# willSapgreen/stereo-vision

Hardware: AMD Instinct MI355X
Metric: stereo pairs/sec (ELAS 1242x375, ROBOTICS, D1+D2+LR) (higher is better)
Workload: dtype u8

## Files before the change

### stereo-vision_amd/csrc/elas_kernels.hip

```cpp
#include <hip/hip_runtime.h>

#include <algorithm>
#include <cstdlib>

#include "dev_common.h"
#include "prior_core.h"
#include "svh_internal.h"

namespace svh {

namespace {

constexpr int kWave = 64;

template <int kCtrl, int kRowMask>
__device__ __forceinline__ uint32_t dpp_min_step(uint32_t v) {
    const uint32_t o =
        (uint32_t)__builtin_amdgcn_update_dpp((int)0xFFFFFFFFu, (int)v, kCtrl, kRowMask, 0xF, false);
    return o < v ? o : v;
}

__device__ __forceinline__ uint32_t wave_min_u32(uint32_t v) {
    v = dpp_min_step<0xB1, 0xF>(v);
    v = dpp_min_step<0x4E, 0xF>(v);
// ... 1679 lines not shown
    __syncthreads();
    float* D = out.D[side] + (size_t)pair * out.stride[side] + (size_t)y * P.DW;
    const int16_t* other = s_raw + (1 - side) * Q.Wr;
    if (P.sub) {
        for (int x = x0; x < P.DW; x += half) {
            const int d = raw_row[x];
            float o = -10.f;
            const float fd = (float)d, step = fd / 2, uwf = side ? (float)x + step : (float)x - step;
            if (d >= 0 && uwf >= 0 && uwf < (float)P.DW)
                if (!(fabsf((float)other[(int)uwf] - fd) > lr_threshold)) o = fd;
            D[x] = o;
        }
        return;
    }
    const int ithr = lr_threshold >= 0.f ? (int)fminf(floorf(lr_threshold), 1048576.f) : -1;
    const uint32_t span = ithr >= 0 ? 2u * (uint32_t)ithr + 1u : 0u;
    const uint32_t raw_a = lds_addr_of(raw_row), oth_a = lds_addr_of(other);
    char* Db = reinterpret_cast<char*>(D);
#define ML_LR_ROW(WARP)                                                                                        \
    _Pragma("unroll") for (int k = 0; k < kIters; k++) {                                                       \
        const int x = x0 + k * half;                                                                           \
        if (x < P.DW) {                                                                                        \
            const int d = (int)(int16_t)lds_read2(raw_a + 2u * (uint32_t)x);                                   \
            const int uw = WARP;                                                                               \
            const int o = (int)(int16_t)lds_read2(oth_a + 2u * (uint32_t)uw);                                  \
            const bool keep = d >= 0 && (uint32_t)uw < (uint32_t)P.DW && (uint32_t)(o - d + ithr) < span;      \
            *reinterpret_cast<float*>(Db + (size_t)(4u * (uint32_t)x)) = keep ? (float)d : -10.f;              \
        }                                                                                                      \
    }
    if (side) { ML_LR_ROW(x + d) } else { ML_LR_ROW(x - d) }
#undef ML_LR_ROW
}

__global__ __launch_bounds__(256) void k_lr(GroupDev G, DevMaps out, int DW, int DH, int sub,
                                            float lr_threshold) {
    const int pair = blockIdx.z;
    const int x = blockIdx.x * 64 + threadIdx.x;
    const int y = blockIdx.y * 4 + threadIdx.y;
    if (x >= DW || y >= DH) return;
    if (!G.hdr->active[pair]) return;
    const size_t DN = (size_t)DW * DH;
    const float* R1 = G.Draw + (size_t)(2 * pair) * DN;
    const float* R2 = R1 + DN;
    float* D1 = out.D[0] + (size_t)pair * out.stride[0];
    float* D2 = out.D[1] + (size_t)pair * out.stride[1];
    const size_t rowo = (size_t)y * DW;
    const float d1 = R1[rowo + x], d2 = R2[rowo + x];
    const float fx = (float)x;
    const float uw1 = sub ? fx - d1 / 2 : fx - d1;
    const float uw2 = sub ? fx + d2 / 2 : fx + d2;
    float o1 = -10.f, o2 = -10.f;
    if (d1 >= 0 && uw1 >= 0 && uw1 < (float)DW)
        if (!(fabsf(R2[rowo + (int)uw1] - d1) > lr_threshold)) o1 = d1;
    if (d2 >= 0 && uw2 >= 0 && uw2 < (float)DW)
        if (!(fabsf(R1[rowo + (int)uw2] - d2) > lr_threshold)) o2 = d2;
    D1[rowo + x] = o1;
    D2[rowo + x] = o2;
}

__device__ __forceinline__ float* post_map(const DevMaps& m, int z, int nside, int* pair) {
    const int p = z / nside, s = z - p * nside;
    *pair = p;
    return m.D[s] + (size_t)p * m.stride[s];
}

__device__ __forceinline__ int uf_find(const int32_t* L, int x) {
    int p = L[x];
    while (p != x) {
        x = p;
        p = L[x];
    }
    return x;
}

__device__ __forceinline__ int uf_find_halve(int32_t* L, int x) {
    int p = L[x];
    while (p != x) {
        const int gp = L[p];
        if (gp != p) L[x] = gp;
        x = p;
        p = gp;
    }
    return x;
}

__device__ __forceinline__ void uf_union(int32_t* L, int a, int b) {
    for (;;) {
        a = uf_find_halve(L, a);
        b = uf_find_halve(L, b);
        if (a == b) return;
        if (a > b) {
            int t = a;
            a = b;
            b = t;
        }
        const int old = atomicMin(&L[b], a);
        if (old == b) return;
        b = old;
    }
}

__device__ __forceinline__ bool seg_joined(float a, float b, float thr) {
    return a >= 0 && b >= 0 && fabsf(a - b) <= thr;
}

constexpr int CX = 64, CY = 16;

__device__ __forceinline__ int lds_find(int* L, int x) {
    int p = __hip_atomic_load(&L[x], __ATOMIC_RELAXED, __HIP_MEMORY_SCOPE_WORKGROUP);
    while (p != x) {
        x = p;
        p = __hip_atomic_load(&L[x], __ATOMIC_RELAXED, __HIP_MEMORY_SCOPE_WORKGROUP);
    }
    return x;
}

__device__ __forceinline__ void lds_union(int* L, int a, int b) {
    for (;;) {
        a = lds_find(L, a);
        b = lds_find(L, b);
        if (a == b) return;
        if (a > b) {
            int t = a;
            a = b;
            b = t;
        }
        const int old = atomicMin(&L[b], a);
        if (old == b) return;
        b = old;
    }
}

struct TileIdx {
    int x, y, z, gx, gy;
};
__device__ __forceinline__ bool tile_index(int tw, int th, int DW, int DH, int nz, TileIdx* t) {
    t->gx = (DW + tw - 1) / tw;
    t->gy = (DH + th - 1) / th;
    if (nz == 0) {
        t->x = blockIdx.x; t->y = blockIdx.y; t->z = blockIdx.z;
        return true;
    }
    const int per = t->gx * t->gy, total = per * nz, chunk = (total + 7) >> 3;
    const int lin = (int)(blockIdx.x & 7) * chunk + (int)(blockIdx.x >> 3);
    if (lin >= total) return false;
    t->z = lin / per;
    const int r = lin - t->z * per;
    t->y = r / t->gx;
    t->x = r - t->y * t->gx;
    return true;
}
inline unsigned xcd_blocks(int total) { return (unsigned)(((total + 7) >> 3) << 3); }

__global__ __launch_bounds__(256) void k_seg_tile(GroupDev G, DevMaps m, PostScratch S, int nside,
                                                  int DW, int DH, float thr, int nz) {
    __shared__ float sD[CY][CX];
    __shared__ int sL[CX * CY];
    __shared__ int sC[CX * CY];
    __shared__ int s_nr;
    TileIdx tb;
    if (!tile_index(CX, CY, DW, DH, nz, &tb)) return;
    int pair;
    const float* D = post_map(m, tb.z, nside, &pair);
    if (!G.hdr->active[pair]) return;
    if (threadIdx.y == 0 && threadIdx.x == 0) s_nr = 0;
    const size_t zo = (size_t)tb.z * DW * DH;
    const int x0 = tb.x * CX, y0 = tb.y * CY;
    const int tx = threadIdx.x;
    int len[CY / 4];
    float dk[CY / 4];
#pragma unroll
    for (int k = 0; k < CY / 4; k++) {
        const int gx = x0 + tx, gy = y0 + (int)threadIdx.y + 4 * k;
        dk[k] = (gx < DW && gy < DH) ? D[gy * DW + gx] : -10.f;
    }
#pragma unroll
    for (int k = 0; k < CY / 4; k++) {
        const int ty = threadIdx.y + 4 * k;
        const float d = dk[k];
        const bool valid = d >= 0;
        const float dl = __shfl_up(d, 1, kWave);
        const bool start = valid && (tx == 0 || !seg_joined(d, dl, thr));
        const unsigned long long starts = __ballot(start);
        const unsigned long long invalid = __ballot(!valid);
        int label = -1;
        len[k] = 0;
        if (valid) {
            const unsigned long long upto = starts & (~0ull >> (63 - tx));
            label = ty * CX + (63 - __clzll((long long)upto));
            if (start) {
                const unsigned long long stops = ((starts | invalid) >> tx) >> 1;
                len[k] = stops ? __ffsll((long long)stops) : (kWave - tx);
            }
        }
        sD[ty][tx] = d;
        sL[ty * CX + tx] = label;
        sC[ty * CX + tx] = 0;
    }
    __syncthreads();
#pragma unroll
    for (int k = 0; k < CY / 4; k++) {
        const int ty = threadIdx.y + 4 * k, i = ty * CX + tx;
        if (ty == 0) continue;
        const float d = sD[ty][tx], du = sD[ty - 1][tx];
        if (!seg_joined(d, du, thr)) continue;
        if (tx > 0) {
            const float dl = sD[ty][tx - 1], dul = sD[ty - 1][tx - 1];
            if (seg_joined(d, dl, thr) && seg_joined(dl, dul, thr) && seg_joined(du, dul, thr)) continue;
        }
        lds_union(sL, sL[i], sL[i - CX]);
    }
    __syncthreads();
#pragma unroll
    for (int k = 0; k < CY / 4; k++) {
        const int ty = threadIdx.y + 4 * k, i = ty * CX + tx;
        if (len[k] > 0) {
            const int r = lds_find(sL, i);
            atomicAdd(&sC[r], len[k]);
            len[k] = r;
        } else {
            len[k] = -1;
        }
    }
    __syncthreads();
#pragma unroll
    for (int k = 0; k < CY / 4; k++)
        if (len[k] >= 0) sL[(threadIdx.y + 4 * k) * CX + tx] = len[k];
    __syncthreads();
#pragma unroll
    for (int k = 0; k < CY / 4; k++) {
        const int ty = threadIdx.y + 4 * k, i = ty * CX + tx;
        const int gx = x0 + tx, gy = y0 + ty;
        if (gx >= DW || gy >= DH) continue;
        const int gi = gy * DW + gx;
        int label = -1, size = 0;
        const int s = sL[i];
        if (s >= 0) {
            const int r = sL[s];
            const int root = sL[r] == r ? r : sL[r];
            const int ry = root / CX, rx = root - ry * CX;
            label = (y0 + ry) * DW + (x0 + rx);
            if (root == i) size = sC[i];
        }
        S.labels[zo + gi] = label;
        if (size > 0) {
            S.counts[zo + gi] = size;
            const int bh = min(CY, DH - y0);
            reinterpret_cast<int32_t*>(S.tmp)[zo + (size_t)y0 * DW + (size_t)x0 * bh + atomicAdd(&s_nr, 1)] = gi;
        }
    }
    __syncthreads();
    if (threadIdx.y == 0 && tx == 0)
        S.nroots[((size_t)tb.z * tb.gy + tb.y) * tb.gx + tb.x] = s_nr;
}

__global__ __launch_bounds__(256) void k_seg_border(GroupDev G, DevMaps m, PostScratch S, int nside,
                                                    int DW, int DH, float thr, int nhor) {
    int pair;
    const float* D = post_map(m, blockIdx.y, nside, &pair);
    if (!G.hdr->active[pair]) return;
    int32_t* L = S.labels + (size_t)blockIdx.y * DW * DH;
    const int e = blockIdx.x * 256 + threadIdx.x;
    int x, y, step;
    if (e < nhor) {
        const int b = e / DW;
        x = e - b * DW;
        y = (b + 1) * CY;
        step = DW;
        if (y >= DH) return;
    } else {
        const int e2 = e - nhor;
        const int nvb = (DW - 1) / CX;
        if (nvb <= 0) return;
        const int b = e2 % nvb;
        y = e2 / nvb;
        x = (b + 1) * CX;
        step = 1;
        if (y >= DH || x >= DW) return;
    }
    const int i = y * DW + x;
    const float d = D[i], q = D[i - step];
    if (!seg_joined(d, q, thr)) return;
    const int along = step == 1 ? DW : 1;
    const bool has_prev = step == 1 ? (y % CY != 0) : (x % CX != 0);
    if (has_prev) {
        const float dp = D[i - along], qp = D[i - step - along];
        if (seg_joined(d, dp, thr) && seg_joined(q, qp, thr) && seg_joined(dp, qp, thr)) return;
    }
    uf_union(L, L[i], L[i - step]);
}

__global__ __launch_bounds__(256) void k_seg_sum(GroupDev G, PostScratch S, int nside, int DW, int DH,
                                                 int min_size) {
    if (!G.hdr->active[blockIdx.y / nside]) return;
    const int n = DW * DH;
    const size_t zo = (size_t)blockIdx.y * n;
    const int tcols = (DW + CX - 1) / CX, trows = (DH + CY - 1) / CY;
    const int tile = blockIdx.x * 4 + (int)(threadIdx.x >> 6), lane = threadIdx.x & 63;
    if (tile >= tcols * trows) return;
    const int ty = tile / tcols, tx = tile - ty * tcols;
    const int y0 = ty * CY, x0 = tx * CX, bh = min(CY, DH - y0);
    const int nroots = S.nroots[(size_t)blockIdx.y * tcols * trows + tile];
    const int32_t* list = reinterpret_cast<const int32_t*>(S.tmp) + zo + (size_t)y0 * DW + (size_t)x0 * bh;
    int32_t* L = S.labels + zo;
    for (int k = lane; k < nroots; k += 64) {
        const int i = list[k];
        const int size = S.counts[zo + i];
        const int root = uf_find(L, i);
        if (root != i) {
            L[i] = root;
            int32_t* c = S.counts + zo + root;
            if (__hip_atomic_load(c, __ATOMIC_RELAXED, __HIP_MEMORY_SCOPE_AGENT) < min_size)
                atomicAdd(c, size);
        }
    }
}

__global__ __launch_bounds__(256) void k_seg_mask(GroupDev G, DevMaps m, PostScratch S, int nside,
                                                  int n, int min_size) {
    const int i = blockIdx.x * 256 + threadIdx.x;
    if (i >= n) return;
    int pair;
    float* D = post_map(m, blockIdx.y, nside, &pair);
    if (!G.hdr->active[pair]) return;
    const size_t zo = (size_t)blockIdx.y * n;
    const int s = S.labels[zo + i];
    if (s < 0) {
        if (1 < min_size) D[i] = -10.f;
    } else if (S.counts[zo + S.labels[zo + s]] < min_size) {
        D[i] = -10.f;
    }
}

__device__ __forceinline__ float gap_value(float d1, float d2) {
    return fabsf(d1 - d2) < 3.0f ? (d1 + d2) / 2 : (d1 < d2 ? d1 : d2);
}

template <bool kCols>
__global__ __launch_bounds__(256) void k_gap_local(GroupDev G, DevMaps m, PostScratch S, int nside,
                                                   int DW, int DH, int gap) {
    const int x = blockIdx.x * 64 + threadIdx.x;
    const int y = blockIdx.y * 4 + threadIdx.y;
    if (x >= DW || y >= DH) return;
    int pair;
    float* D = post_map(m, blockIdx.z, nside, &pair);
    if (!G.hdr->active[pair]) return;
    float* tmp = S.tmp + (size_t)blockIdx.z * DW * DH;
    const float* in = kCols ? tmp : D;
    float* out = kCols ? D : tmp;
    const int i = y * DW + x;
    const int stride = kCols ? DW : 1;
    const int pos = kCols ? y : x, len = kCols ? DH : DW;
    float val = in[i];
    if (!(val >= 0)) {
        if (gap <= 4) {
            float nl[4], nr[4];
#pragma unroll
            for (int k = 1; k <= 4; k++) {
                nl[k - 1] = (k <= gap && pos - k >= 0) ? in[i - k * stride] : -1.f;
                nr[k - 1] = (k <= gap && pos + k < len) ? in[i + k * stride] : -1.f;
            }
            int l = 0, r = 0;
            float vl = 0.f, vr = 0.f;
#pragma unroll
            for (int k = 4; k >= 1; k--) {
                if (nl[k - 1] >= 0) { l = k; vl = nl[k - 1]; }
                if (nr[k - 1] >= 0) { r = k; vr = nr[k - 1]; }
            }
            if (l && r && r <= gap - l + 1) val = gap_value(vl, vr);
        } else {
            int l = 0, r = 0;
            for (int k = 1; k <= gap && pos - k >= 0; k++)
                if (in[i - k * stride] >= 0) {
                    l = k;
                    break;
                }
            if (l) {
                for (int k = 1; k <= gap - l + 1 && pos + k < len; k++)
                    if (in[i + k * stride] >= 0) {
                        r = k;
                        break;
                    }
                if (r) val = gap_value(in[i - l * stride], in[i + r * stride]);
            }
        }
    }
    out[i] = val;
}

template <bool kCols>
__global__ void k_gap_lines(GroupDev G, DevMaps m, int nside, int DW, int DH, int gap,
                            int add_corners) {
    const int line = blockIdx.x * blockDim.x + threadIdx.x;
    const int nlines = kCols ? DW : DH;
    if (line >= nlines) return;
    int pair;
    float* D = post_map(m, blockIdx.y, nside, &pair);
    if (!G.hdr->active[pair]) return;
    const int len = kCols ? DH : DW;
    const int stride = kCols ? DW : 1;
    float* base = D + (kCols ? line : (size_t)line * DW);
    int count = 0;
    for (int p = 0; p < len; p++) {
        if (base[(size_t)p * stride] >= 0) {
            if (count >= 1 && count <= gap) {
                const int first = p - count, last = p - 1;
                if (first > 0 && last < len - 1) {
                    const float di = gap_value(base[(size_t)(first - 1) * stride],
                                               base[(size_t)(last + 1) * stride]);
                    for (int q = first; q <= last; q++) base[(size_t)q * stride] = di;
                }
            }
            count = 0;
        } else {
            count++;
        }
    }
    if (add_corners) {
        for (int p = 0; p < len; p++)
            if (base[(size_t)p * stride] >= 0) {
                const float val = base[(size_t)p * stride];
                for (int q = (p - gap > 0 ? p - gap : 0); q < p; q++) base[(size_t)q * stride] = val;
                break;
            }
        for (int p = len - 1; p >= 0; p--)
            if (base[(size_t)p * stride] >= 0) {
                const float val = base[(size_t)p * stride];
                const int qe = p + gap < len - 1 ? p + gap : len - 1;
                for (int q = p; q <= qe; q++) base[(size_t)q * stride] = val;
                break;
            }
    }
}

constexpr int kGapChunks = 48;
__global__ __launch_bounds__(256) void k_gap_rows_scan(GroupDev G, DevMaps m, int nside, int DW, int DH, int gap,
                                                       int add_corners) {
    extern __shared__ float s_gapline[];
    __shared__ unsigned long long s_mask[4][kGapChunks];
    __shared__ int s_prev[4][kGapChunks], s_next[4][kGapChunks];
    const int lane = threadIdx.x & 63, wave = __builtin_amdgcn_readfirstlane((int)(threadIdx.x >> 6));
    const int row = blockIdx.x * 4 + wave;
    if (row >= DH) return;
    int pair;
    float* D = post_map(m, blockIdx.y, nside, &pair);
    if (!G.hdr->active[pair]) return;
    float* base = D + (size_t)row * DW;
    const int nch = (DW + 63) >> 6;
    float* line = s_gapline + wave * (nch * 64);
    constexpr int kNone = 1 << 30;
    int run = -1;
    for (int k = 0; k < nch; k++) {
        const int p = 64 * k + lane;
        const float v = p < DW ? base[p] : -1.f;
        line[p] = v;
        const unsigned long long mk = __builtin_amdgcn_ballot_w64(v >= 0);
        s_mask[wave][k] = mk;
        s_prev[wave][k] = run;
        if (mk) run = 64 * k + 63 - __builtin_clzll(mk);
    }
    const int pl = run;
    int runn = kNone;
    for (int k = nch - 1; k >= 0; k--) {
        const unsigned long long mk = s_mask[wave][k];
        s_next[wave][k] = runn;
        if (mk) runn = 64 * k + __builtin_ctzll(mk);
    }
    const int pf = runn;
    __builtin_amdgcn_wave_barrier();
    for (int k = 0; k < nch; k++) {
        const int p = 64 * k + lane;
        const float v = line[p];
        if (p >= DW || v >= 0) continue;
        const unsigned long long mk = s_mask[wave][k];
        const unsigned long long lower = mk & ((1ull << lane) - 1ull), upper = mk >> lane;
        const int L = lower ? 64 * k + 63 - __builtin_clzll(lower) : s_prev[wave][k];
        const int R = upper ? p + __builtin_ctzll(upper) : s_next[wave][k];
        float o = v;
        if (L >= 0 && R != kNone) {
            if (R - L - 1 <= gap) o = gap_value(line[L], line[R]);
        } else if (add_corners) {
            if (L < 0 && R != kNone && p >= pf - gap) o = line[pf];
// ... 321 lines not shown
    Q.Ws = ((d.W + 3) & ~3) + 2;
    static const bool wide768 = !(svh::env("SVH_MATCH_WIDE768") && atoi(svh::env("SVH_MATCH_WIDE768")) == 0);
    int iters = (d.DW + 255) / 256;
    Q.half = std::min(256, ((d.DW + iters - 1) / iters + 63) / 64 * 64);
    if (iters > 5 && wide768 && d.DW <= 5 * 384) {
        iters = (d.DW + 383) / 384;
        Q.half = std::min(384, ((d.DW + iters - 1) / iters + 63) / 64 * 64);
    }
    Q.kIters = iters <= 5 ? 5 : 8;
    static const bool xcd_rows = !(svh::env("SVH_MATCH_XCD") && atoi(svh::env("SVH_MATCH_XCD")) == 0);
    Q.xcd = xcd_rows ? 1 : 0;
    const size_t ldsl = (size_t)2 * Q.Ws * sizeof(uint4) + (size_t)2 * d.gw * ML_CAP * sizeof(uint16_t) +
                        (size_t)2 * Q.Wr * sizeof(int16_t);
    constexpr size_t kListStatic = 256;
    bool ok = ldsl + kListStatic <= 160 * 1024;
    if (ok && ldsl + kListStatic > 64 * 1024) {
        ok = hipFuncSetAttribute((const void*)k_match_list<true, 5>, hipFuncAttributeMaxDynamicSharedMemorySize,
                                 160 * 1024 - (int)kListStatic) == hipSuccess &&
             hipFuncSetAttribute((const void*)k_match_list<false, 5>, hipFuncAttributeMaxDynamicSharedMemorySize,
                                 160 * 1024 - (int)kListStatic) == hipSuccess &&
             hipFuncSetAttribute((const void*)k_match_list<true, 8>, hipFuncAttributeMaxDynamicSharedMemorySize,
                                 160 * 1024 - (int)kListStatic) == hipSuccess &&
             hipFuncSetAttribute((const void*)k_match_list<false, 8>, hipFuncAttributeMaxDynamicSharedMemorySize,
                                 160 * 1024 - (int)kListStatic) == hipSuccess;
        if (!ok) (void)hipGetLastError();
    }
    if (Qout) *Qout = Q;
    if (lds_out) *lds_out = ldsl;
    return ok;
}

static bool match_keyed_usable(const svh_elas_params& p, const Dims& d, int32_t prior_absmax, int32_t plane_radius,
                               bool with_lr, size_t* lds2_out) {
    static const bool ordered = svh::env("SVH_MATCH_ORDERED") != nullptr;
    const bool keyed_ok = !ordered && prior_absmax < (1 << 19) && p.disp_max < 512 && plane_radius <= 15 &&
                          d.W < 65536 && p.grid_size > 1;
    const size_t lds = (size_t)d.W * sizeof(uint4);
    const size_t lds2 = 2 * lds + (with_lr ? (size_t)2 * d.DW * sizeof(float) : 0);
    if (lds2_out) *lds2_out = lds2;
    constexpr size_t keyed_lds_max = 96 * 1024;
    constexpr size_t kStaticLds = 64 * sizeof(int);
    bool use_keyed = keyed_ok && lds2 + kStaticLds <= keyed_lds_max;
    if (use_keyed && lds2 + kStaticLds > 64 * 1024) {
        use_keyed = hipFuncSetAttribute((const void*)k_match_keyed<true>, hipFuncAttributeMaxDynamicSharedMemorySize,
                                        (int)keyed_lds_max) == hipSuccess &&
                    hipFuncSetAttribute((const void*)k_match_keyed<false>, hipFuncAttributeMaxDynamicSharedMemorySize,
                                        (int)keyed_lds_max) == hipSuccess;
        if (!use_keyed) (void)hipGetLastError();
    }
    return use_keyed;
}

bool descriptors_on_the_fly(const svh_elas_params& p, const Dims& d, int32_t prior_absmax, int32_t plane_radius,
                            bool have_lists) {
    static const bool off = svh::env("SVH_DESC_FLY") && atoi(svh::env("SVH_DESC_FLY")) == 0;
    static const bool keyed_fly = !(svh::env("SVH_DESC_FLY_KEYED") && atoi(svh::env("SVH_DESC_FLY_KEYED")) == 0);
    if (off || d.W < 8 || support_strip(p, d, nullptr) == 0) return false;
    if (match_list_usable(p, d, prior_absmax, plane_radius, have_lists, nullptr, nullptr)) return true;
    return keyed_fly && match_keyed_usable(p, d, prior_absmax, plane_radius, true, nullptr);
}

bool launch_match(const LaunchCtx& cx, const svh_elas_params& p, const Dims& d, int32_t g,
                  const GroupDev& G, const DevMaps* lr_out, bool write_raw, const char** error) {
    if (error) *error = nullptr;
    MatchParams P;
    P.W = d.W; P.H = d.H; P.DW = d.DW; P.DH = d.DH; P.gw = d.gw; P.gh = d.gh; P.gwords = d.gwords;
    P.grid_size = p.grid_size; P.sub = p.subsampling; P.disp_max = p.disp_max;
    P.match_texture = p.match_texture; P.plane_radius = G.plane_radius;
    P.grid_magic = (uint32_t)(0x100000000ull / (uint64_t)p.grid_size) + 1u;
    P.npairs = g;
    const size_t lds = (size_t)d.W * sizeof(uint4);
    constexpr size_t kStaticLds = 64 * sizeof(int);
    size_t lds2 = 0;
    const bool use_keyed = match_keyed_usable(p, d, G.prior_absmax, G.plane_radius, lr_out != nullptr, &lds2);
    {
        MatchList Q{};
        size_t ldsl = 0;
        const bool ok = match_list_usable(p, d, G.prior_absmax, G.plane_radius, G.lists != nullptr, &Q, &ldsl);
        const int half = Q.half;
        if (!ok && !use_keyed && G.desc_fly) {
            if (error) *error = "both row matchers were refused after the descriptor stage had left only the Sobel planes";
            return false;
        }
        if (ok) {
            Timed timed_(cx, "k_match");
            const dim3 grid((unsigned)(Q.xcd ? (d.DH * g + 7) / 8 * 8 : d.DH * g)), block(2 * half);
            hipStream_t s = (hipStream_t)cx.stream;
            DevMaps none{};
            const DevMaps& o = lr_out ? *lr_out : none;
            const int wr = lr_out ? (write_raw ? 1 : 0) : 1;
            const float thr = lr_out ? (float)p.lr_threshold : 0.f;
            if (lr_out) {
                if (Q.kIters == 5) hipLaunchKernelGGL((k_match_list<true, 5>), grid, block, ldsl, s, G, P, Q, o, wr, thr);
                else hipLaunchKernelGGL((k_match_list<true, 8>), grid, block, ldsl, s, G, P, Q, o, wr, thr);
                return true;
            }
            if (Q.kIters == 5) hipLaunchKernelGGL((k_match_list<false, 5>), grid, block, ldsl, s, G, P, Q, o, wr, thr);
            else hipLaunchKernelGGL((k_match_list<false, 8>), grid, block, ldsl, s, G, P, Q, o, wr, thr);
            return false;
        }
    }
    if (use_keyed) {
        Timed timed_(cx, "k_match");
        static const int mt = std::min(256, std::max(64, svh::env("SVH_MATCH_THREADS") ? atoi(svh::env("SVH_MATCH_THREADS")) : 256));
        const int iters = (d.DW + mt - 1) / mt;
        const int half = std::min(256, ((d.DW + iters - 1) / iters + 63) / 64 * 64);
        const dim3 grid(xcd_blocks(d.DH * g)), block(2 * half);
        hipStream_t s = (hipStream_t)cx.stream;
        if (lr_out) {
            hipLaunchKernelGGL(k_match_keyed<true>, grid, block, lds2, s, G, P, *lr_out, write_raw ? 1 : 0,
                               (float)p.lr_threshold);
            return true;
        }
        DevMaps none{};
        hipLaunchKernelGGL(k_match_keyed<false>, grid, block, lds2, s, G, P, none, 1, 0.f);
    } else if (lds + kStaticLds <= 64 * 1024) {
        Timed timed_(cx, "k_match");
        static const int mt = svh::env("SVH_MATCH_THREADS") ? atoi(svh::env("SVH_MATCH_THREADS")) : 256;
        const int iters = (d.DW + mt - 1) / mt;
        const int threads = std::min(512, ((d.DW + iters - 1) / iters + 63) / 64 * 64);
        hipLaunchKernelGGL(k_match<true>, dim3(1, d.DH, 2 * g), dim3(threads), lds,
                           (hipStream_t)cx.stream, G, P);
    } else {
        LAUNCH("k_match", k_match<false>, grid2d(d.DW, d.DH, 2 * g), dim3(64, 4), G, P);
    }
    return false;
}

void launch_lr(const LaunchCtx& cx, const svh_elas_params& p, const Dims& d, int32_t g,
               const GroupDev& G, const DevMaps& out) {
    LAUNCH("k_lr", k_lr, grid2d(d.DW, d.DH, g), dim3(64, 4), G, out, d.DW, d.DH, p.subsampling,
           (float)p.lr_threshold);
}

void launch_segments(const LaunchCtx& cx, const svh_elas_params& p, const Dims& d, int32_t g,
                     int32_t nside, const GroupDev& G, const DevMaps& out, const PostScratch& S, bool mask) {
    const int n = d.DW * d.DH, z = g * nside;
    int min_size = p.speckle_size;
    if (p.subsampling) min_size = (int)(sqrtf((float)p.speckle_size) * 2);
    const dim3 lin((n + 255) / 256, z), b256(256);
    launch_segments_label(cx, p, d, g, nside, G, out, S);
    if (mask) LAUNCH("k_seg_mask", k_seg_mask, lin, b256, G, out, S, nside, n, min_size);
}


void launch_segments_label(const LaunchCtx& cx, const svh_elas_params& p, const Dims& d, int32_t g,
                           int32_t nside, const GroupDev& G, const DevMaps& in, const PostScratch& S) {
    const int n = d.DW * d.DH, z = g * nside;
    int min_size = p.speckle_size;
    if (p.subsampling) min_size = (int)(sqrtf((float)p.speckle_size) * 2);
    const dim3 lin((n + 255) / 256, z), b256(256);
    const dim3 tiles((d.DW + CX - 1) / CX, (d.DH + CY - 1) / CY, z);
    static const bool tile_xcd = !(svh::env("SVH_TILE_XCD") && atoi(svh::env("SVH_TILE_XCD")) == 0);
    if (tile_xcd)
        LAUNCH("k_seg_tile", k_seg_tile, dim3(xcd_blocks((int)(tiles.x * tiles.y * tiles.z))), dim3(CX, 4), G, in, S, nside,
               d.DW, d.DH, p.speckle_sim_threshold, z);
    else
        LAUNCH("k_seg_tile", k_seg_tile, tiles, dim3(CX, 4), G, in, S, nside, d.DW, d.DH,
               p.speckle_sim_threshold, 0);
    const int nhor = ((d.DH - 1) / CY) * d.DW;
    const int nver = ((d.DW - 1) / CX) * d.DH;
    if (nhor + nver > 0)
        LAUNCH("k_seg_border", k_seg_border, dim3((nhor + nver + 255) / 256, z), b256, G, in, S, nside,
               d.DW, d.DH, p.speckle_sim_threshold, nhor);
    LAUNCH("k_seg_sum", k_seg_sum, dim3((tiles.x * tiles.y + 3) / 4, z), b256, G, S, nside, d.DW, d.DH, min_size);
}


void launch_gap(const LaunchCtx& cx, const svh_elas_params& p, const Dims& d, int32_t g,
                int32_t nside, const GroupDev& G, const DevMaps& out, const PostScratch& S) {
    int gap = p.ipol_gap_width;
    if (p.subsampling) gap = p.ipol_gap_width / 2 + 1;
    const int z = g * nside;
    if (gap <= 16 && !p.add_corners) {
        LAUNCH("k_gap_rows", k_gap_local<false>, grid2d(d.DW, d.DH, z), dim3(64, 4), G, out, S, nside,
               d.DW, d.DH, gap);
        LAUNCH("k_gap_cols", k_gap_local<true>, grid2d(d.DW, d.DH, z), dim3(64, 4), G, out, S, nside,
               d.DW, d.DH, gap);
    } else {
        static const bool seq = svh::env("SVH_GAP_SEQ") && atoi(svh::env("SVH_GAP_SEQ")) != 0;
        const int nch = (d.DW + 63) / 64;
        if (!seq && nch <= kGapChunks) {
            {
                Timed timed_(cx, "k_gap_rows_scan");
                hipLaunchKernelGGL(k_gap_rows_scan, dim3((d.DH + 3) / 4, z), dim3(256), (size_t)4 * nch * 64 * sizeof(float),
                                   (hipStream_t)cx.stream, G, out, nside, d.DW, d.DH, gap, (int)p.add_corners);
            }
            LAUNCH("k_gap_cols_seg", k_gap_cols_seg, dim3((d.DW + 63) / 64, z), dim3(64, kGapSeg), G, out,
                   nside, d.DW, d.DH, gap, p.add_corners);
            return;
        }
        LAUNCH("k_gap_rows_seq", k_gap_lines<false>, dim3((d.DH + 63) / 64, z), dim3(64), G, out,
               nside, d.DW, d.DH, gap, p.add_corners);
        LAUNCH("k_gap_cols_seq", k_gap_lines<true>, dim3((d.DW + 63) / 64, z), dim3(64), G, out,
               nside, d.DW, d.DH, gap, p.add_corners);
    }
}

constexpr int QX = 64, QY = 32;

__device__ __forceinline__ float gap_pick(float val, const float* line, int stride, int pos, int len, int gap) {
    float a[4], b[4];
#pragma unroll
    for (int k = 1; k <= 4; k++) {
        a[k - 1] = line[-k * stride];
        b[k - 1] = line[k * stride];
    }
    asm volatile("" ::: "memory");
    if (val >= 0) return val;
    int l = 0, r = 0;
    float vl = 0.f, vr = 0.f;
#pragma unroll
    for (int k = 4; k >= 1; k--) {
        if (k <= gap && pos - k >= 0 && a[k - 1] >= 0) { l = k; vl = a[k - 1]; }
        if (k <= gap && pos + k < len && b[k - 1] >= 0) { r = k; vr = b[k - 1]; }
    }
    return (l && r && r <= gap - l + 1) ? gap_value(vl, vr) : val;
}

__global__ __launch_bounds__(256) void k_gap_tile(GroupDev G, DevMaps m, PostScratch S, int nside, int DW,
                                                  int DH, int gap, int min_size, int nz) {
    constexpr int HG = 4;
    __shared__ float sA[QY + 2 * HG][QX + 2 * HG];
    __shared__ float sB[QY + 2 * HG][QX];
    TileIdx tb;
    if (!tile_index(QX, QY, DW, DH, nz, &tb)) return;
    int pair;
    const float* D = post_map(m, tb.z, nside, &pair);
    if (!G.hdr->active[pair]) return;
    float* out = S.tmp + (size_t)tb.z * DW * DH;
    const int x0 = tb.x * QX, y0 = tb.y * QY;
    const int tid = threadIdx.y * 64 + threadIdx.x;
    {
        constexpr int AW = QX + 2 * HG, AH = QY + 2 * HG, NR = AH / 4, NE = NR + (AH * 8 + 255) / 256;
        static_assert(AH % 4 == 0 && AW - 64 == 8, "tile shape");
        const int32_t* L = S.labels + (size_t)tb.z * DW * DH;
        const int32_t* Cn = S.counts + (size_t)tb.z * DW * DH;
        const int lane = threadIdx.x, wave = __builtin_amdgcn_readfirstlane(threadIdx.y);
        float val[NE];
        int lab[NE];
        int er[NE], ec[NE];
#pragma unroll
        for (int k = 0; k < NE; k++) {
            if (k < NR) {
                er[k] = wave + 4 * k;
                ec[k] = lane;
            } else {
                const int e = tid + 256 * (k - NR);
                er[k] = e >> 3;
                ec[k] = 64 + (e & 7);
            }
            const int gy = y0 - HG + er[k], gx = x0 - HG + ec[k];
            const bool in = er[k] < AH && gy >= 0 && gy < DH && gx >= 0 && gx < DW;
            val[k] = in ? D[(size_t)gy * DW + gx] : -10.f;
            lab[k] = (in && min_size > 0) ? L[(size_t)gy * DW + gx] : -1;
        }
        if (min_size > 0) {
#pragma unroll
            for (int k = 0; k < NE; k++)
                if (lab[k] >= 0) lab[k] = L[lab[k]];
#pragma unroll
            for (int k = 0; k < NE; k++)
                if (lab[k] >= 0 && Cn[lab[k]] < min_size) val[k] = -10.f;
        }
#pragma unroll
        for (int k = 0; k < NE; k++)
            if (er[k] < AH) sA[er[k]][ec[k]] = val[k];
    }
    __syncthreads();
    for (int i = tid; i < (QY + 2 * HG) * QX; i += 256) {
        const int r = i >> 6, c = i & 63;
        const int gx = x0 + c;
        sB[r][c] = gx < DW ? gap_pick(sA[r][c + HG], &sA[r][c + HG], 1, gx, DW, gap) : -10.f;
    }
    __syncthreads();
    for (int i = tid; i < QY * QX; i += 256) {
        const int r = i >> 6, c = i & 63;
        const int gy = y0 + r, gx = x0 + c;
        if (gy < DH && gx < DW)
            out[(size_t)gy * DW + gx] = gap_pick(sB[r + HG][c], &sB[r + HG][c], QX, gy, DH, gap);
    }
}

__device__ __forceinline__ float am_weight_q(float val, float centre) {
    const float mm = __uint_as_float(__float_as_uint(__fsub_rn(val, centre)) & 0x4F000000u);
    return __builtin_amdgcn_fmed3f(__fmaf_rn(mm, -0.25f, 1.0f), 0.0f, 1.0f);
}

template <int kTaps, int kRot, typename Tap>
__device__ __forceinline__ bool am_eval_rot(Tap tap, float centre, float* res) {
    constexpr int kCentre = kTaps == 8 ? 4 : 2;
    float P[4], F[4];
#pragma unroll
    for (int m = 0; m < 4; m++) {
        float w0 = 1.0f, f0 = centre;
        if (m != kCentre) {
            const float t0 = tap(m);
            w0 = am_weight_q(t0, centre);
            f0 = __fmul_rn(t0, w0);
        }
        if (kTaps == 8) {
            float w1 = 1.0f, f1 = centre;
            if (m + 4 != kCentre) {
                const float t1 = tap(m + 4);
                w1 = am_weight_q(t1, centre);
                f1 = __fmul_rn(t1, w1);
            }
            P[m] = __fadd_rn(w0, w1);
            F[m] = __fadd_rn(f0, f1);
        } else {
            P[m] = w0;
            F[m] = f0;
        }
    }
    constexpr int a = (4 - kRot) & 3;
    const float wsum = __fadd_rn(__fadd_rn(__fadd_rn(P[a], P[(a + 1) & 3]), P[(a + 2) & 3]), P[(a + 3) & 3]);
    const float fsum = __fadd_rn(__fadd_rn(__fadd_rn(F[a], F[(a + 1) & 3]), F[(a + 2) & 3]), F[(a + 3) & 3]);
    if (wsum > 0) {
        const float dv = __fdiv_rn(fsum, wsum);
        if (dv >= 0) {
            *res = dv;
            return true;
        }
    }
    return false;
}

constexpr int kMeanSub = 20, kMeanSA = 80, kMeanSB = 65;

template <int kTaps, int kQ>
__device__ __forceinline__ void mean_row_pass(const float* sA, float* sB, int x0, int y0, int DW, int DH,
                                              int lane) {
    constexpr int back = kTaps == 8 ? 3 : 1, lead = kTaps - 1, HL = lead - back, HR = back;
    constexpr int AH = QY + HL + HR;
    const int l = lane & 15, rs = lane >> 4;
    const int gx = x0 + 4 * l + kQ;
    const bool xin = gx >= lead - back && gx <= DW - 1 - back;
    const float* a = sA + rs * kMeanSA + l;
    float* b = sB + rs * kMeanSB + 4 * l + kQ;
#pragma unroll 2
    for (int r4 = 0; r4 < AH; r4 += 4) {
        const int r = r4 + rs;
        if (r < AH) {
            const int gy = y0 - HL + r;
            const float* row = a + r4 * kMeanSA;
            const float centre = row[((kQ + HL) & 3) * kMeanSub + ((kQ + HL) >> 2)];
            float res = centre < 0 ? -10.f : 0.f;
            if (centre >= 0 && xin && gy >= 3 && gy < DH - 3)
                am_eval_rot<kTaps, (kQ - HL) & 3>(
                    [&](int k) { return row[((kQ + k) & 3) * kMeanSub + ((kQ + k) >> 2)]; }, centre, &res);
            b[r4 * kMeanSB] = res;
        }
    }
}

template <int kTaps, int kQ>
__device__ __forceinline__ void mean_col_pass(const float* sB, float* D, const float (&orig)[QY / 4], int x0,
                                              int y0, int DW, int DH, int lane) {
    constexpr int back = kTaps == 8 ? 3 : 1, lead = kTaps - 1, HL = lead - back;
    const int gx = x0 + lane;
    if (gx >= DW) return;
    const bool xin = gx >= 3 && gx < DW - 3;
#pragma unroll
    for (int j = 0; j < QY / 4; j++) {
        const int r = kQ + 4 * j, gy = y0 + r;
        if (gy >= DH) break;
        const float* col = sB + r * kMeanSB + lane;
        float res = orig[j];
        const float centre = col[HL * kMeanSB];
        if (centre >= 0 && xin && gy >= lead - back && gy <= DH - 1 - back)
            am_eval_rot<kTaps, (kQ - HL) & 3>([&](int k) { return col[k * kMeanSB]; }, centre, &res);
        D[(size_t)gy * DW + gx] = res;
    }
}

template <int kTaps>
__global__ __launch_bounds__(256) void k_mean_tile(GroupDev G, DevMaps m, PostScratch S, int nside, int DW,
                                                   int DH, int nz) {
    constexpr int back = kTaps == 8 ? 3 : 1, lead = kTaps - 1;
    constexpr int HL = lead - back, HR = back;
    constexpr int AW = QX + HL + HR, AH = QY + HL + HR;
    static_assert((AW + 3) / 4 <= kMeanSub && 4 * kMeanSub <= kMeanSA && QX <= kMeanSB, "tile layout");
    __shared__ float sA[AH * kMeanSA];
    __shared__ float sB[AH * kMeanSB];
    TileIdx tb;
    if (!tile_index(QX, QY, DW, DH, nz, &tb)) return;
    int pair;
    float* D = post_map(m, tb.z, nside, &pair);
    if (!G.hdr->active[pair]) return;
    const float* in = S.tmp + (size_t)tb.z * DW * DH;
    const int x0 = tb.x * QX, y0 = tb.y * QY;
    const int lane = threadIdx.x;
    const int wave = __builtin_amdgcn_readfirstlane(threadIdx.y);
    float orig[QY / 4];
    {
        constexpr int NR = (AH + 3) / 4, XW = AW - 64, NX = (AH * XW + 255) / 256;
        float val[NR], xv[NX];
        const int gxm = x0 - HL + lane;
        const bool cin = gxm >= 0 && gxm < DW;
#pragma unroll
        for (int j = 0; j < NR; j++) {
            const int r = wave + 4 * j, gy = y0 - HL + r;
            val[j] = (r < AH && gy >= 0 && gy < DH && cin) ? in[(size_t)gy * DW + gxm] : -10.f;
        }
        const int tid = wave * 64 + lane;
#pragma unroll
        for (int k = 0; k < NX; k++) {
            const int e = tid + 256 * k, r = e / XW, c = 64 + (e - r * XW);
            const int gy = y0 - HL + r, gx = x0 - HL + c;
            xv[k] = (e < AH * XW && gy >= 0 && gy < DH && gx < DW) ? in[(size_t)gy * DW + gx] : -10.f;
        }
#pragma unroll
        for (int j = 0; j < QY / 4; j++) {
            const int gy = y0 + wave + 4 * j, gx = x0 + lane;
            orig[j] = (gy < DH && gx < DW) ? in[(size_t)gy * DW + gx] : 0.f;
        }
// ... 83 lines not shown
```

Before: 38710.

## Settle speckle segments inside tiles to skip global union-find work

The tile segmentation kernel now tags each component with whether it touches a tile border, using a high bit packed into the LDS size counter. Components already at least min_size get a keep sentinel, and interior components smaller than min_size get a remove sentinel, so they skip the global root list, border unions and label indirections. Border and sum kernels treat sentinel neighbours by saturating counts with atomicMax, and the fused gap/mask kernel skips the dependent label/count gathers when no lane in a wave needs them. This adds sentinel logic and changes the counting semantics, so correctness depends on the saturation handling being consistent.

```diff
diff --git a/stereo-vision_amd/csrc/elas_kernels.hip b/stereo-vision_amd/csrc/elas_kernels.hip
--- a/stereo-vision_amd/csrc/elas_kernels.hip
+++ b/stereo-vision_amd/csrc/elas_kernels.hip
@@ -1855,8 +1855,11 @@
 }
 inline unsigned xcd_blocks(int total) { return (unsigned)(((total + 7) >> 3) << 3); }
 
+constexpr int kSegInvalid = -1, kSegKeep = -2, kSegRemove = -3;
+constexpr int kSegTouch = 1 << 16;
+
 __global__ __launch_bounds__(256) void k_seg_tile(GroupDev G, DevMaps m, PostScratch S, int nside,
-                                                  int DW, int DH, float thr, int nz) {
+                                                  int DW, int DH, float thr, int min_size, int nz) {
     __shared__ float sD[CY][CX];
     __shared__ int sL[CX * CY];
     __shared__ int sC[CX * CY];
@@ -1919,7 +1922,9 @@
         const int ty = threadIdx.y + 4 * k, i = ty * CX + tx;
         if (len[k] > 0) {
             const int r = lds_find(sL, i);
-            atomicAdd(&sC[r], len[k]);
+            const bool touch = (ty == 0 && y0 > 0) || (ty == CY - 1 && y0 + CY < DH) ||
+                               (tx == 0 && x0 > 0) || (tx + len[k] == CX && x0 + CX < DW);
+            atomicAdd(&sC[r], len[k] + (touch ? kSegTouch : 0));
             len[k] = r;
         } else {
             len[k] = -1;
@@ -1936,14 +1941,21 @@
         const int gx = x0 + tx, gy = y0 + ty;
         if (gx >= DW || gy >= DH) continue;
         const int gi = gy * DW + gx;
-        int label = -1, size = 0;
+        int label = kSegInvalid, size = 0;
         const int s = sL[i];
         if (s >= 0) {
             const int r = sL[s];
             const int root = sL[r] == r ? r : sL[r];
-            const int ry = root / CX, rx = root - ry * CX;
-            label = (y0 + ry) * DW + (x0 + rx);
-            if (root == i) size = sC[i];
+            const int word = sC[root], n = word & (kSegTouch - 1);
+            if (min_size > 0 && n >= min_size) {
+                label = kSegKeep;
+            } else if (min_size > 0 && word < kSegTouch) {
+                label = kSegRemove;
+            } else {
+                const int ry = root / CX, rx = root - ry * CX;
+                label = (y0 + ry) * DW + (x0 + rx);
+                if (root == i) size = n;
+            }
         }
         S.labels[zo + gi] = label;
         if (size > 0) {
@@ -1958,7 +1970,7 @@
 }
 
 __global__ __launch_bounds__(256) void k_seg_border(GroupDev G, DevMaps m, PostScratch S, int nside,
-                                                    int DW, int DH, float thr, int nhor) {
+                                                    int DW, int DH, float thr, int nhor, int min_size) {
     int pair;
     const float* D = post_map(m, blockIdx.y, nside, &pair);
     if (!G.hdr->active[pair]) return;
@@ -1982,15 +1994,22 @@
         if (y >= DH || x >= DW) return;
     }
     const int i = y * DW + x;
+    const int la = L[i], lb = L[i - step];
+    if (la == kSegInvalid || lb == kSegInvalid) return;
+    if (la < 0 && lb < 0) return;
     const float d = D[i], q = D[i - step];
     if (!seg_joined(d, q, thr)) return;
+    if (la < 0 || lb < 0) {
+        atomicMax(S.counts + (size_t)blockIdx.y * DW * DH + (la < 0 ? lb : la), min_size);
+        return;
+    }
     const int along = step == 1 ? DW : 1;
     const bool has_prev = step == 1 ? (y % CY != 0) : (x % CX != 0);
     if (has_prev) {
         const float dp = D[i - along], qp = D[i - step - along];
         if (seg_joined(d, dp, thr) && seg_joined(q, qp, thr) && seg_joined(dp, qp, thr)) return;
     }
-    uf_union(L, L[i], L[i - step]);
+    uf_union(L, la, lb);
 }
 
 __global__ __launch_bounds__(256) void k_seg_sum(GroupDev G, PostScratch S, int nside, int DW, int DH,
@@ -2013,8 +2032,10 @@
         if (root != i) {
             L[i] = root;
             int32_t* c = S.counts + zo + root;
-            if (__hip_atomic_load(c, __ATOMIC_RELAXED, __HIP_MEMORY_SCOPE_AGENT) < min_size)
-                atomicAdd(c, size);
+            if (__hip_atomic_load(c, __ATOMIC_RELAXED, __HIP_MEMORY_SCOPE_AGENT) < min_size) {
+                if (size >= min_size) atomicMax(c, min_size);
+                else atomicAdd(c, size);
+            }
         }
     }
 }
@@ -2028,9 +2049,11 @@
     if (!G.hdr->active[pair]) return;
     const size_t zo = (size_t)blockIdx.y * n;
     const int s = S.labels[zo + i];
-    if (s < 0) {
+    if (s == kSegInvalid) {
         if (1 < min_size) D[i] = -10.f;
-    } else if (S.counts[zo + S.labels[zo + s]] < min_size) {
+    } else if (s == kSegRemove) {
+        D[i] = -10.f;
+    } else if (s >= 0 && S.counts[zo + S.labels[zo + s]] < min_size) {
         D[i] = -10.f;
     }
 }
@@ -2658,17 +2681,19 @@
     const dim3 lin((n + 255) / 256, z), b256(256);
     const dim3 tiles((d.DW + CX - 1) / CX, (d.DH + CY - 1) / CY, z);
     static const bool tile_xcd = !(svh::env("SVH_TILE_XCD") && atoi(svh::env("SVH_TILE_XCD")) == 0);
+    static const bool settle = !(svh::env("SVH_SEG_SETTLE") && atoi(svh::env("SVH_SEG_SETTLE")) == 0);
+    const int tile_min = settle ? std::max(min_size, 1) : 0;
     if (tile_xcd)
         LAUNCH("k_seg_tile", k_seg_tile, dim3(xcd_blocks((int)(tiles.x * tiles.y * tiles.z))), dim3(CX, 4), G, in, S, nside,
-               d.DW, d.DH, p.speckle_sim_threshold, z);
+               d.DW, d.DH, p.speckle_sim_threshold, tile_min, z);
     else
         LAUNCH("k_seg_tile", k_seg_tile, tiles, dim3(CX, 4), G, in, S, nside, d.DW, d.DH,
-               p.speckle_sim_threshold, 0);
+               p.speckle_sim_threshold, tile_min, 0);
     const int nhor = ((d.DH - 1) / CY) * d.DW;
     const int nver = ((d.DW - 1) / CX) * d.DH;
     if (nhor + nver > 0)
         LAUNCH("k_seg_border", k_seg_border, dim3((nhor + nver + 255) / 256, z), b256, G, in, S, nside,
-               d.DW, d.DH, p.speckle_sim_threshold, nhor);
+               d.DW, d.DH, p.speckle_sim_threshold, nhor, min_size);
     LAUNCH("k_seg_sum", k_seg_sum, dim3((tiles.x * tiles.y + 3) / 4, z), b256, G, S, nside, d.DW, d.DH, min_size);
 }
 
@@ -2759,15 +2784,23 @@
             const int gy = y0 - HG + er[k], gx = x0 - HG + ec[k];
             const bool in = er[k] < AH && gy >= 0 && gy < DH && gx >= 0 && gx < DW;
             val[k] = in ? D[(size_t)gy * DW + gx] : -10.f;
-            lab[k] = (in && min_size > 0) ? L[(size_t)gy * DW + gx] : -1;
+            lab[k] = (in && min_size > 0) ? L[(size_t)gy * DW + gx] : kSegInvalid;
         }
         if (min_size > 0) {
-#pragma unroll
-            for (int k = 0; k < NE; k++)
-                if (lab[k] >= 0) lab[k] = L[lab[k]];
-#pragma unroll
-            for (int k = 0; k < NE; k++)
-                if (lab[k] >= 0 && Cn[lab[k]] < min_size) val[k] = -10.f;
+            bool need = false;
+#pragma unroll
+            for (int k = 0; k < NE; k++) {
+                if (lab[k] == kSegRemove) val[k] = -10.f;
+                need |= lab[k] >= 0;
+            }
+            if (__any(need)) {
+#pragma unroll
+                for (int k = 0; k < NE; k++)
+                    if (lab[k] >= 0) lab[k] = L[lab[k]];
+#pragma unroll
+                for (int k = 0; k < NE; k++)
+                    if (lab[k] >= 0 && Cn[lab[k]] < min_size) val[k] = -10.f;
+            }
         }
 #pragma unroll
         for (int k = 0; k < NE; k++)
```

New measurement: 39500 (median of 6 runs). 1.02x the previous value.
